# LucasAlegre/morl-baselines

Hardware: NVIDIA H100
Metric: envelope_q_updates_per_sec (higher is better)
Workload: dtype f32

## Files before the change

include/morl_b200.h:

```cpp
#ifndef MORL_B200_H_
#define MORL_B200_H_

#include <stddef.h>
#include <stdint.h>

#ifdef __cplusplus
extern "C" {
#endif

#define MORL_B200_VERSION 100

#if defined(__GNUC__)
#define MORL_API __attribute__((visibility("default")))
#else
#define MORL_API
#endif

#define MORL_OK 0
#define MORL_ERR_NULL (-1)
#define MORL_ERR_SHAPE (-2)
#define MORL_ERR_ALIGN (-3)
#define MORL_ERR_UNSUPPORTED (-4)
#define MORL_ERR_NO_DEVICE (-5)

// ... 110 lines not shown
MORL_API int morl_gemm_planes_f32(int fmt, const void* a_planes, long long a_plane_stride, const float* a_scale, const void* b_planes,
                                  long long b_plane_stride, const float* b_scale, int M, int N, int N_pad, int K, const float* bias,
                                  int relu, const void* relu_mask_plane0, int ld_mask, float* c_f32, int ldc, void* c_planes, int ldp,
                                  long long c_plane_stride, const float* c_scale, int reverse_tiles, int split_accumulators,
                                  const void* relu_bits_in, void* relu_bits_out, void* stream);
MORL_API int morl_gemm_planes_ln_f32(int fmt, const void* a_planes, long long a_plane_stride, const float* a_scale, const void* b_planes,
                                     long long b_plane_stride, const float* b_scale, int M, int N, int K, const float* bias, int layer_norm,
                                     const float* ln_gamma, const float* ln_beta, float ln_eps, float drop_p, const unsigned long long* drop_seed,
                                     const unsigned int* drop_offset, unsigned int drop_salt, float* c_f32, int ldc, void* c_planes, int ldp,
                                     long long c_plane_stride, const float* c_scale, int reverse_tiles, void* drop_bits_out, void* stream);
MORL_API int morl_philox_advance(unsigned int* offset, unsigned int inc, void* stream);
MORL_API int morl_gemm_chain_supported(int fmt, int M, int K);
MORL_API int morl_gemm_chain_f32(int fmt, int n_chains, int n_layers, const void* const* act_planes, long long act_plane_stride, const float* act_scale,
                                 const void* const* w_planes, long long w_plane_stride, const float* const* w_scales, const float* const* biases,
                                 int relu, const void* const* relu_bits_in, void* const* relu_bits_out, int M, int K, int k_first, void* stream);
MORL_API int morl_debug_gemm_stats(unsigned long long* out8, int reset);
MORL_API int morl_ensemble_sample_f32(const float* out, const float* max_logvar, const float* min_logvar, const int32_t* model_idx, const float* noise,
                                      const float* obs, int rew_dim, int E, int N, int O, float* sample_out, float* var_out, float* uncertainty_out,
                                      void* stream);

MORL_API int morl_qhead_envelope_supported(int fmt, int B, int W, int A, int D, int K);
MORL_API int morl_qhead_gemm_supported(int fmt, int M, int N, int K);
MORL_API int morl_qhead_gemm_f32(int fmt, const void* a_planes, long long a_plane_stride, const float* a_scale, const void* w_planes,
                                 long long w_plane_stride, const float* w_scale, const float* bias, int M, int N, int K, int reverse_tiles,
                                 float* q_out, void* stream);
MORL_API int morl_qhead_envelope_td_f32(int fmt, const void* a_on_planes, const void* a_tg_planes, long long a_plane_stride,
                                        const float* a_scale_on, const float* a_scale_tg, const void* w_on_planes, const void* w_tg_planes,
                                        long long w_plane_stride, const float* w_scale_on, const float* w_scale_tg, const float* bias_on,
                                        const float* bias_tg, int K, const float* wset, const float* reward, const float* done, float gamma,
                                        int B, int W, int A, int D, int dot_mode, int row_order, int reverse_tiles, float* target_out,
// ... 37 lines not shown
```

morl_baselines_b200/_lib.py:

```python

from __future__ import annotations

import ctypes as C
import os

HERE = os.path.dirname(os.path.abspath(__file__))
LIB_PATH = os.path.join(HERE, "csrc", "libmorl_b200.so")

DOT_UNFUSED, DOT_FMA, DOT_PAIRFMA = 0, 1, 2
MAP_TILE, MAP_BLOCK = 0, 1
ROWS_REFERENCE, ROWS_BMAJOR = 0, 1
AC_ELEMENTWISE_MIN, AC_SCALAR_MIN, AC_ARGMIN_GATHER = 0, 1, 2
MAX_D = 8
FMT_BF16X3, FMT_F16X2 = 0, 1

_vp, _i, _f, _d, _i64, _sz = C.c_void_p, C.c_int, C.c_float, C.c_double, C.c_int64, C.c_size_t

SIGNATURES = {
    "morl_version": (_i, []),
    "morl_last_error": (C.c_char_p, []),
    "morl_device_sm_count": (_i, []),
    "morl_envelope_td_f32": (_i, [_vp, _vp, _vp, _vp, _vp, _f, _i, _i, _i, _i, _i, _i, _vp, _vp, _vp, _vp]),
    "morl_greedy_td_f32": (_i, [_vp, _vp, _vp, _i, _i, _vp, _vp, _i, _i, _f, _i, _i, _i, _i, _vp, _vp, _vp]),
    "morl_critic_min_td_f32": (_i, [_vp, _i, _vp, _i, _i, _vp, _vp, _i, _i, _f, _i, _i, _i, _i, _vp, _vp, _vp]),
# ... 20 lines not shown
    "morl_front_unpack_f64": (_i, [_vp, _i, _i, _i, _i, _vp, _vp, _vp]),
    "morl_hypervolume_f64": (_i, [_vp, _vp, _i, _i, _vp, _vp, _vp]),
    "morl_corner_weights_f64": (_i, [_vp, _i, _i, _vp, _i, _vp, _vp]),
    "morl_polyak_f32": (_i, [_vp, _vp, _vp, _i, _i64, _d, _vp]),
    "morl_plane_overflow_count": (_i, [_i]),
    "morl_amax_scale_f32": (_i, [_vp, C.c_longlong, _i, _vp, _vp, _vp]),
    "morl_split_planes_multi": (_i, [_i, _vp, _i, _vp]),
    "morl_split_planes": (_i, [_i, _vp, _i, _i, _i, _i, _vp, _i, _i, C.c_longlong, _vp, _vp]),
    "morl_gemm_planes_f32": (_i, [_i, _vp, C.c_longlong, _vp, _vp, C.c_longlong, _vp, _i, _i, _i, _i, _vp, _i, _vp, _i, _vp, _i, _vp, _i, C.c_longlong,
                                  _vp, _i, _i, _vp, _vp, _vp]),
    "morl_gemm_planes_ln_f32": (_i, [_i, _vp, C.c_longlong, _vp, _vp, C.c_longlong, _vp, _i, _i, _i, _vp, _i, _vp, _vp, _f, _f, _vp, _vp, C.c_uint,
                                     _vp, _i, _vp, _i, C.c_longlong, _vp, _i, _vp, _vp]),
    "morl_philox_advance": (_i, [_vp, C.c_uint, _vp]),
    "morl_gemm_chain_supported": (_i, [_i, _i, _i]),
    "morl_gemm_chain_f32": (_i, [_i, _i, _i, _vp, C.c_longlong, _vp, _vp, C.c_longlong, _vp, _vp, _i, _vp, _vp, _i, _i, _i, _vp]),
    "morl_debug_gemm_stats": (_i, [_vp, _i]),
    "morl_ensemble_sample_f32": (_i, [_vp, _vp, _vp, _vp, _vp, _vp, _i, _i, _i, _i, _vp, _vp, _vp, _vp]),
    "morl_qhead_envelope_supported": (_i, [_i, _i, _i, _i, _i, _i]),
    "morl_qhead_gemm_supported": (_i, [_i, _i, _i, _i]),
    "morl_qhead_gemm_f32": (_i, [_i, _vp, C.c_longlong, _vp, _vp, C.c_longlong, _vp, _vp, _i, _i, _i, _i, _vp, _vp]),
    "morl_qhead_envelope_td_f32": (_i, [_i, _vp, _vp, C.c_longlong, _vp, _vp, _vp, _vp, C.c_longlong, _vp, _vp, _vp, _vp, _i, _vp, _vp, _vp, _f, _i, _i,
                                        _i, _i, _i, _i, _i, _vp, _vp, _vp, _vp, _vp, _vp]),
    "morl_pairs_relu_split_planes": (_i, [_i, _vp, _vp, _i, _i, _i, _vp, C.c_longlong, _vp, _vp, _vp]),
    "morl_pairs_product_split_planes": (_i, [_i, _vp, _vp, _i, _i, _i, _vp, C.c_longlong, _vp, _vp]),
    "morl_gemm_mn_workspace_bytes": (_sz, [_i, _i, _i]),
    "morl_gemm_planes_mn_f32": (_i, [_i, _vp, C.c_longlong, _i, _i, _vp, _vp, C.c_longlong, _i, _i, _vp, _i, _i, _vp, _i, _vp, _vp, _vp]),
    "morl_colsum_planes": (_i, [_i, _vp, C.c_longlong, _vp, _i, _i, _i, _vp, _vp, _vp]),
    "morl_pairs_grad_reduce_planes": (_i, [_i, _vp, C.c_longlong, _vp, _i, _i, _i, _vp, _vp, _vp, _vp]),
    "morl_pair_layer1_uv_f32": (_i, [_vp, _vp, _vp, _vp, _i, _i, _i, _i, _i, _vp, _vp, _vp]),
    "morl_product_layer1_uv_f32": (_i, [_vp, _vp, _vp, _i, _i, _vp, _vp, _vp, _i, _i, _i, _vp, _vp, _vp]),
# ... 45 lines not shown
```

morl_baselines_b200/csrc/gemm_planes.cu:

```cuda
#include <cuda.h>
#include <cuda_bf16.h>
#include <cuda_fp16.h>
#include <stdlib.h>
#include <string.h>

#include "common.cuh"
#include "gemm_tc.cuh"

namespace morl {

constexpr int kGemmBM = 128;
constexpr int kGemmThreads = 384;
constexpr int kGemmConsumerRegs = 232, kGemmProducerRegs = 40;
constexpr int kGemmBoxN = 32;

__device__ unsigned int g_plane_overflow;


__device__ __forceinline__ void note_overflow(float amax) {
    if (amax > 65504.f) atomicAdd(&g_plane_overflow, 1u);
}

#define MORL_DISPATCH_FMT(F_, ...)                                                         \
    switch (F_) {                                                                          \
// ... 163 lines not shown
    float k_acc;
    float c_mul;
    const float* bias_s;
    int relu;
    const uint32_t* bits_in;
    uint32_t* bits_out;
    int bits_ld;
    const uint16_t* mask;
    int ld_mask;
    float* c_f32;
    int ldc;
    int planes;
    int ldp;
};

template <int FMT, bool PRE = false>
__device__ __forceinline__ void epilogue_chunk(const float (&a)[16], int col0, int rbase, int lane, const EpiArgs& e, const CUtensorMap* tmC,
                                               uint8_t* my_stage, uint32_t& n_stored, float& amax) {
    using F = PlaneFmt<FMT>;
    constexpr int P = F::P;
    const int l4 = lane & 3, lr = lane >> 2;
    const int wi = relu_bits_word(col0);
    float x[2][8];
#pragma unroll
    for (int h = 0; h < 2; ++h)
#pragma unroll
        for (int q = 0; q < 4; ++q)
#pragma unroll
            for (int c = 0; c < 2; ++c) {
                float f;
                if constexpr (PRE) f = a[4 * q + 2 * h + c];
                else f = __fmaf_rn(a[4 * q + 2 * h + c], e.k_acc, e.bias_s[col0 + 8 * q + 2 * l4 + c]);
                if (e.relu) f = (f < 0.f) ? 0.f : f;
                x[h][2 * q + c] = f;
            }
    if (e.bits_in) {
#pragma unroll
        for (int h = 0; h < 2; ++h) {
            const int row = rbase + lr + 8 * h;
            const uint32_t keep = row < e.M ? __ldg(e.bits_in + (size_t)row * e.bits_ld + wi) : 0u;
#pragma unroll
            for (int j = 0; j < 8; ++j)
                if (!((keep >> (8 * (j >> 1) + 2 * l4 + (j & 1))) & 1u)) x[h][j] = 0.f;
        }
    }
    if (e.bits_out) {
#pragma unroll
        for (int h = 0; h < 2; ++h) {
            const int row = rbase + lr + 8 * h;
            uint32_t positive = 0;
#pragma unroll
            for (int j = 0; j < 8; ++j)
                if (x[h][j] > 0.f) positive |= 1u << (8 * (j >> 1) + 2 * l4 + (j & 1));
            positive |= __shfl_xor_sync(0xffffffffu, positive, 1);
            positive |= __shfl_xor_sync(0xffffffffu, positive, 2);
            if (l4 == 0 && row < e.M) e.bits_out[(size_t)row * e.bits_ld + wi] = positive;
        }
    }
    if (e.mask) {
#pragma unroll
        for (int h = 0; h < 2; ++h) {
            const int row = rbase + lr + 8 * h;
            if (row < e.M) {
#pragma unroll
                for (int q = 0; q < 4; ++q) {
                    const uint32_t mm = __ldg(reinterpret_cast<const uint32_t*>(e.mask + (size_t)row * e.ld_mask + col0 + 8 * q + 2 * l4));
                    if ((mm & 0x8000u) || (mm & 0x7FFFu) == 0u) x[h][2 * q] = 0.f;
                    if ((mm & 0x80000000u) || (mm & 0x7FFF0000u) == 0u) x[h][2 * q + 1] = 0.f;
                }
            }
        }
    }
    if (e.c_f32) {
// ... 354 lines not shown
                    e.k_acc = s_act / (s_act * ld_scale(g.b_scale[job]));
                    e.c_mul = 1.0f;
                    e.bias_s = s.bias; e.relu = g.relu; e.bits_in = g.bits_in[job]; e.bits_out = g.bits_out[job]; e.bits_ld = relu_bits_words(BN);
                    e.mask = nullptr; e.ld_mask = 0;
                    e.c_f32 = nullptr; e.ldc = 0; e.planes = 1; e.ldp = BN;
                    const int rbase = tile * kGemmBM + wg * 64 + (warp & 3) * 16;
                    consume_unit<FMT, 0, false>(acc, s, ring, l == 0 ? n_kblk_first : n_kblk_full, 0, BN, rbase, wg, lane, nullptr, [] {}, e,
                                                &maps.C[job], my_stage, n_stored, amax);
                    __syncwarp();
                    if (lane == 0) {
                        asm volatile("cp.async.bulk.wait_group 0;" ::: "memory");
                        g_mbar_arrive(&stored[ln]);
                    }
                }
        if (FMT == MORL_FMT_F16X2) note_overflow(amax);
    }
}

constexpr int kMnKT = 32;

__device__ __forceinline__ uint64_t make_desc_mn_sw128(uint32_t smem_addr, uint32_t lbo_bytes) {
    uint64_t d = 0;
    d |= (uint64_t)((smem_addr >> 4) & 0x3FFF);
    d |= (uint64_t)((lbo_bytes >> 4) & 0x3FFF) << 16;
    d |= (uint64_t)(1024 >> 4) << 32;
    d |= (uint64_t)1 << 62;
    return d;
}

struct GemmMnArgs {
// ... 1079 lines not shown
    a.thr = t >= 4294967295.0 ? 4294967295u : (unsigned int)t;
    a.scale = (float)(1.0 / (1.0 - (double)drop_p));
    a.bits = drop_bits_out;
    return gemm_planes_impl(fmt, a_planes, a_plane_stride, a_scale, b_planes, b_plane_stride, b_scale, M, N, N, K, bias, 1, nullptr, 0, c_f32, ldc,
                            c_planes, ldp, c_plane_stride, c_scale, reverse_tiles, 0, nullptr, nullptr, &a, "morl_gemm_planes_ln_f32", stream);
}

extern "C" int morl_philox_advance(unsigned int* offset, unsigned int inc, void* stream) {
    using namespace morl;
    MORL_REQUIRE(offset, MORL_ERR_NULL, "morl_philox_advance: NULL pointer argument");
    launch_k(philox_advance_kernel, dim3(1), dim3(1), 0, static_cast<cudaStream_t>(stream), offset, inc);
    return check_launch("morl_philox_advance");
}


extern "C" int morl_gemm_chain_supported(int fmt, int M, int K) {
    using namespace morl;
    return fmt_ok(fmt) && M >= 2 * kGemmBM && K == 256;
}

extern "C" int morl_gemm_chain_f32(int fmt, int n_chains, int n_layers, const void* const* act_planes, long long act_plane_stride, const float* act_scale,
                                   const void* const* w_planes, long long w_plane_stride, const float* const* w_scales, const float* const* biases,
                                   int relu, const void* const* relu_bits_in, void* const* relu_bits_out, int M, int K, int k_first, void* stream) {
    using namespace morl;
    MORL_REQUIRE(act_planes && w_planes, MORL_ERR_NULL, "morl_gemm_chain_f32: NULL pointer argument");
    MORL_REQUIRE(n_chains >= 1 && n_chains <= 2 && n_layers >= 1 && n_chains * n_layers <= kChainMaxJobs, MORL_ERR_SHAPE,
                 "morl_gemm_chain_f32: need 1 <= n_chains <= 2 and n_chains * n_layers <= %d (got %d x %d)", kChainMaxJobs, n_chains, n_layers);
    MORL_REQUIRE(morl_gemm_chain_supported(fmt, M, K), MORL_ERR_UNSUPPORTED, "morl_gemm_chain_f32: unsupported configuration fmt=%d M=%d K=%d (256-wide layers, M >= 256)",
                 fmt, M, K);
    const int BK = fmt_bk(fmt);
    if (k_first <= 0) k_first = K;
    MORL_REQUIRE(k_first % BK == 0 && k_first <= K, MORL_ERR_SHAPE, "morl_gemm_chain_f32: k_first=%d must be a multiple of %d and <= K", k_first, BK);
    ChainMaps maps;
    ChainArgs g;
    memset(&g, 0, sizeof(g));
    g.M = M; g.K = K; g.k_first = k_first; g.n_chains = n_chains; g.n_layers = n_layers; g.a_scale = act_scale; g.relu = relu ? 1 : 0;
    for (int c = 0; c < n_chains; ++c)
        for (int l = 0; l < n_layers; ++l) {
            const int job = c * n_layers + l;
            const void* a_in = act_planes[c * (n_layers + 1) + l];
            const void* a_out = act_planes[c * (n_layers + 1) + l + 1];
            MORL_REQUIRE(a_in && a_out && w_planes[job] && aligned16(a_in) && aligned16(a_out) && aligned16(w_planes[job]), MORL_ERR_NULL,
                         "morl_gemm_chain_f32: NULL or misaligned plane pointer (chain %d, layer %d)", c, l);
            const int kj = l == 0 ? k_first : K;
            const long long a_stride = l == 0 ? (long long)M * k_first : act_plane_stride;
            const long long w_stride = l == 0 ? (long long)256 * k_first : w_plane_stride;
            int rc = make_plane_map(&maps.A[job], fmt, a_in, M, kj, a_stride, kGemmBM, BK);
// ... 7 lines not shown
            g.bits_out[job] = relu_bits_out ? static_cast<uint32_t*>(relu_bits_out[job]) : nullptr;
            g.bits_in[job] = relu_bits_in ? static_cast<const uint32_t*>(relu_bits_in[job]) : nullptr;
            MORL_REQUIRE(aligned16(g.bits_out[job]) && aligned16(g.bits_in[job]), MORL_ERR_ALIGN, "morl_gemm_chain_f32: ReLU bit masks must be 16-byte aligned");
        }
    const int sms = sm_count();
    const int n_tiles = (M + kGemmBM - 1) / kGemmBM;
    MORL_DISPATCH_FMT(fmt, {
        constexpr size_t smem = KPlan<kFmt>::kBytes;
        g.n_stages = KPlan<kFmt>::kStages;
        set_smem_limit_once<gemm_chain_kernel<kFmt>>(smem);
        launch_k_pdl(gemm_pdl_enabled(), gemm_chain_kernel<kFmt>, dim3(n_tiles < sms ? n_tiles : sms), dim3(kGemmThreads), smem,
                     static_cast<cudaStream_t>(stream), maps, g);
    });
    return check_launch("morl_gemm_chain_f32");
}
```

morl_baselines_b200/multi_policy/envelope/envelope.py:

```python

from __future__ import annotations

import os
from typing import List, Optional, Union

import numpy as np
import torch as th
import torch.nn as nn
import torch.optim as optim

from ... import ops
from ...tc_mlp import TCPairMlp, TCPairMlpFn
from ...common.buffer import ReplayBuffer
from ...common.fused_adam import FusedClipAdam
from ...common.morl_algorithm import MOAgent, MOPolicy
from ...common.networks import NatureCNN, get_grad_norm, layer_init, mlp, polyak_update
from ...common.prioritized_buffer import PrioritizedReplayBuffer
from ...common.utils import linearly_decaying_value
from ...common.weights import equally_spaced_weights, random_weights

_FUSED_HEAD = os.environ.get("MORL_FUSED_HEAD", "1") != "0"
_PRE_REFRESH = os.environ.get("MORL_PRE_REFRESH", "1") == "1"
_HEAD_REVERSE = os.environ.get("MORL_HEAD_REVERSE", "1") == "1"
_DEFER_TREE = os.environ.get("MORL_DEFER_TREE", "1") != "0"
# ... 319 lines not shown
                else:
                    TCPairMlp.refresh_many([self._tc_on, self._tc_tg], transposed_of=[self._tc_train] if self._tc_train is not None else [])
                early_q = None
                if _THREE_STREAMS and self._tc_train is not None:
                    main, side3 = th.cuda.current_stream(), s["side_stream3"]
                    side3.wait_stream(main)
                    with th.cuda.stream(side3):
                        dp_ = self._dp
                        ws_ = wset if dp_ is None else wset[dp_["rank"] * dp_["w_loc"] : (dp_["rank"] + 1) * dp_["w_loc"]]
                        early_q = self._tc_train.forward_pairs(obs, ws_)
                fused_head = self.envelope and _FUSED_HEAD and self.tensor_core_accumulators != "split" and self._tc_on.head_operands() is not None \
                    and ops.qhead_envelope_supported(self._tc_fmt, B, W, A, D, self._tc_on.lin[-1].in_features)
                self.fused_head_active = bool(fused_head)
                head_reverse = False
                if fused_head:
                    if self._tc_on.chain_supported() and self._tc_tg.chain_supported():
                        if self._nograd_chain is None:
                            self._nograd_chain = TCPairMlp.make_chain([self._tc_on, self._tc_tg])
                        self._tc_on.layer1(nobs, wset)
                        self._tc_tg.layer1(nobs, wset)
                        self._nograd_chain()
                        h_on, h_tg = self._tc_on.h[-1], self._tc_tg.h[-1]
                        head_reverse = _HEAD_REVERSE
                    elif _TWO_STREAMS:
                        main, side = th.cuda.current_stream(), s["side_stream2"]
                        side.wait_stream(main)
                        with th.cuda.stream(side):
                            h_tg = self._tc_tg.forward_hidden(nobs, wset)
                        h_on = self._tc_on.forward_hidden(nobs, wset)
                        main.wait_stream(side)
                    else:
# ... 422 lines not shown
```

morl_baselines_b200/ops.py:

```python

from __future__ import annotations

from typing import Optional, Tuple

import torch as th

from . import _lib
from ._lib import (
    AC_ARGMIN_GATHER,
    AC_ELEMENTWISE_MIN,
    AC_SCALAR_MIN,
    DOT_FMA,
    DOT_PAIRFMA,
    DOT_UNFUSED,
    MAP_BLOCK,
    MAP_TILE,
    ROWS_BMAJOR,
    ROWS_REFERENCE,
)

launch_count = 0


def _count(n=1):
# ... 589 lines not shown
            if t is not None and (t.dtype != th.int32 or tuple(t.shape) != (self.M, relu_bits_words(self.N)) or not t.is_contiguous()):
                raise _lib.MorlB200Error(f"GemmChain: ReLU bit masks must be contiguous int32 [{self.M}, {relu_bits_words(self.N)}]")
        self._keep = (flat_a, flat_w, flat_b, flat_s, flat_m, flat_i, act_scale)
        self.relu = bool(relu)
        arr = lambda ts: (C.c_void_p * len(ts))(*[None if t is None else t.data_ptr() for t in ts])
        self._pa, self._pw, self._pb, self._ps, self._pm, self._pi = arr(flat_a), arr(flat_w), arr(flat_b), arr(flat_s), arr(flat_m), arr(flat_i)
        self._a_stride, self._w_stride, self._act_scale = a0.stride(0), 256 * self.K, act_scale

    def __call__(self):
        rc = _lib.load().morl_gemm_chain_f32(self.fmt, self.n_chains, self.n_layers, self._pa, self._a_stride, _ptr(self._act_scale), self._pw, self._w_stride,
                                             self._ps, self._pb, int(self.relu), self._pi, self._pm, self.M, self.K, self.k_first, _stream())
        _lib.check(rc, "morl_gemm_chain_f32")
        _count()


def qhead_gemm_supported(fmt: int, M: int, N: int, K: int) -> bool:
    return bool(_lib.load().morl_qhead_gemm_supported(int(fmt), int(M), int(N), int(K)))


def qhead_gemm(a_planes: th.Tensor, w_planes: th.Tensor, n_out: int, bias: th.Tensor, out: Optional[th.Tensor] = None, a_scale=None, w_scale=None,
               reverse_tiles: bool = False) -> th.Tensor:
    fmt = fmt_of(a_planes)
    _, M, K = a_planes.shape
    if fmt_of(w_planes) != fmt or tuple(w_planes.shape[1:]) != (32, K) or a_planes.stride(1) != K or w_planes.stride(1) != K:
        raise _lib.MorlB200Error(f"qhead_gemm: need K-major planes A [P, M, K] and W [P, 32, K] of one format (got {tuple(a_planes.shape)}, {tuple(w_planes.shape)})")
    if out is None:
        out = th.empty((M, n_out), device=a_planes.device, dtype=th.float32)
    rc = _lib.load().morl_qhead_gemm_f32(fmt, _ptr(a_planes), a_planes.stride(0), _ptr(a_scale), _ptr(w_planes), w_planes.stride(0), _ptr(w_scale), _ptr(bias), M,
                                         n_out, K, int(reverse_tiles), _ptr(out), _stream())
    _lib.check(rc, "morl_qhead_gemm_f32")
# ... 169 lines not shown
```

morl_baselines_b200/tc_mlp.py:

```python

from __future__ import annotations

import os
from typing import List, Optional

import torch as th
from torch import nn

from . import ops

_SNAKE = os.environ.get("MORL_TC_SNAKE", "1") == "1"
_CHAIN = os.environ.get("MORL_GEMM_CHAIN", "1") == "1"
_CHAIN_BWD = os.environ.get("MORL_GEMM_CHAIN_BWD", "1") == "1"
_NARROW_HEAD = os.environ.get("MORL_NARROW_HEAD", "1") == "1"
_DEFAULT_FMT = ops.FMT_BF16X3 if os.environ.get("MORL_TC_FMT", "f16x2") == "bf16x3" else ops.FMT_F16X2

MAX_HIDDEN = 512
MAX_TRAIN_W = 256
ACT_SCALE = 2.0
W_TARGET_EXP = 14
G_TARGET_EXP = 2


def _pad(n: int, m: int) -> int:
# ... 137 lines not shown
                                   reverse_tiles=_SNAKE and bool(k & 1), a_scale=self.s_act, b_scale=self.s_w[k - 1], c_scale=self.s_act,
                                   split_acc=self.split_acc, relu_bits_out=hb[k])
        return a

    def chain_supported(self) -> bool:
        hid = [l.out_features for l in self.lin[:-1]]
        return (_CHAIN and not self.split_acc and len(hid) >= 2 and all(h == 256 for h in hid)
                and ops.gemm_chain_supported(self.fmt, self.B * self.W, 256))

    def layer1(self, feats: th.Tensor, wset: th.Tensor) -> th.Tensor:
        first = self.lin[0]
        u, v = ops.pair_layer1_uv(feats, wset, first.weight.detach(), first.bias.detach())
        hb = self.hbits if self.trainable else [None] * len(self.h)
        return ops.pairs_relu_split(u, v, out=self.h[0], scale=self.s_act, relu_bits_out=hb[0])

    def chain_spec(self):
        n = len(self.lin)
        hb = self.hbits if self.trainable else [None] * len(self.h)
        return (list(self.h), [self.wp[k - 1] for k in range(1, n - 1)], [self.lin[k].bias for k in range(1, n - 1)],
                [self.s_w[k - 1] for k in range(1, n - 1)], [hb[k] for k in range(1, n - 1)])

    @staticmethod
    def make_chain(plans):
        specs = [p.chain_spec() for p in plans]
        return ops.GemmChain([sp[0] for sp in specs], [sp[1] for sp in specs], [sp[2] for sp in specs], [sp[3] for sp in specs],
                             [sp[4] for sp in specs], act_scale=plans[0].s_act)

    def head_operands(self):
        last = self.lin[-1]
        wp = self.wp[len(self.lin) - 2]
# ... 208 lines not shown
```

Before: 693.7.

## Fuse pair-expansion layer into a shared-memory-resident GEMM chain kernel

Adds a persistent chain kernel that builds the first hidden activation (relu(u[b]+v[j])) directly in shared memory from the per-observation and per-weight partial products, then runs all hidden 256-wide layers with the activation kept resident in shared memory. Only the last layer's output is written to global memory. This removes the separate pairs_relu_split pass and the global write and reload of intermediate activation planes. It is used on the no-grad target path when the format is f16x2. In exchange it adds a large new kernel with a 3-stage weight ring and extra shared-memory pressure.

```diff
diff --git a/include/morl_b200.h b/include/morl_b200.h
--- a/include/morl_b200.h
+++ b/include/morl_b200.h
@@ -148,6 +148,10 @@
 MORL_API int morl_gemm_chain_f32(int fmt, int n_chains, int n_layers, const void* const* act_planes, long long act_plane_stride, const float* act_scale,
                                  const void* const* w_planes, long long w_plane_stride, const float* const* w_scales, const float* const* biases,
                                  int relu, const void* const* relu_bits_in, void* const* relu_bits_out, int M, int K, int k_first, void* stream);
+MORL_API int morl_gemm_chain_pairs_f32(int n_chains, int n_layers, const float* const* u, const float* const* v, int B, int W, const void* const* acts,
+                                       long long act_plane_stride, const float* act_scale, const void* const* w_planes, long long w_plane_stride,
+                                       const float* const* w_scales, const float* const* biases, void* const* relu_bits_out, unsigned int store_mask,
+                                       void* stream);
 MORL_API int morl_debug_gemm_stats(unsigned long long* out8, int reset);
 MORL_API int morl_ensemble_sample_f32(const float* out, const float* max_logvar, const float* min_logvar, const int32_t* model_idx, const float* noise,
                                       const float* obs, int rew_dim, int E, int N, int O, float* sample_out, float* var_out, float* uncertainty_out,
diff --git a/morl_baselines_b200/_lib.py b/morl_baselines_b200/_lib.py
--- a/morl_baselines_b200/_lib.py
+++ b/morl_baselines_b200/_lib.py
@@ -58,6 +58,7 @@
     "morl_philox_advance": (_i, [_vp, C.c_uint, _vp]),
     "morl_gemm_chain_supported": (_i, [_i, _i, _i]),
     "morl_gemm_chain_f32": (_i, [_i, _i, _i, _vp, C.c_longlong, _vp, _vp, C.c_longlong, _vp, _vp, _i, _vp, _vp, _i, _i, _i, _vp]),
+    "morl_gemm_chain_pairs_f32": (_i, [_i, _i, _vp, _vp, _i, _i, _vp, C.c_longlong, _vp, _vp, C.c_longlong, _vp, _vp, _vp, C.c_uint, _vp]),
     "morl_debug_gemm_stats": (_i, [_vp, _i]),
     "morl_ensemble_sample_f32": (_i, [_vp, _vp, _vp, _vp, _vp, _vp, _i, _i, _i, _i, _vp, _vp, _vp, _vp]),
     "morl_qhead_envelope_supported": (_i, [_i, _i, _i, _i, _i, _i]),
diff --git a/morl_baselines_b200/csrc/gemm_planes.cu b/morl_baselines_b200/csrc/gemm_planes.cu
--- a/morl_baselines_b200/csrc/gemm_planes.cu
+++ b/morl_baselines_b200/csrc/gemm_planes.cu
@@ -201,49 +201,55 @@
     int ldp;
 };
 
+template <bool PRE>
+__device__ __forceinline__ void epilogue_values(const float (&a)[16], int col0, int rbase, int lane, const EpiArgs& e, float (&x)[2][8]) {
+    const int l4 = lane & 3, lr = lane >> 2;
+    const int wi = relu_bits_word(col0);
+#pragma unroll
+    for (int h = 0; h < 2; ++h)
+#pragma unroll
+        for (int q = 0; q < 4; ++q)
+#pragma unroll
+            for (int c = 0; c < 2; ++c) {
+                float f;
+                if constexpr (PRE) f = a[4 * q + 2 * h + c];
+                else f = __fmaf_rn(a[4 * q + 2 * h + c], e.k_acc, e.bias_s[col0 + 8 * q + 2 * l4 + c]);
+                if (e.relu) f = (f < 0.f) ? 0.f : f;
+                x[h][2 * q + c] = f;
+            }
+    if (e.bits_in) {
+#pragma unroll
+        for (int h = 0; h < 2; ++h) {
+            const int row = rbase + lr + 8 * h;
+            const uint32_t keep = row < e.M ? __ldg(e.bits_in + (size_t)row * e.bits_ld + wi) : 0u;
+#pragma unroll
+            for (int j = 0; j < 8; ++j)
+                if (!((keep >> (8 * (j >> 1) + 2 * l4 + (j & 1))) & 1u)) x[h][j] = 0.f;
+        }
+    }
+    if (e.bits_out) {
+#pragma unroll
+        for (int h = 0; h < 2; ++h) {
+            const int row = rbase + lr + 8 * h;
+            uint32_t positive = 0;
+#pragma unroll
+            for (int j = 0; j < 8; ++j)
+                if (x[h][j] > 0.f) positive |= 1u << (8 * (j >> 1) + 2 * l4 + (j & 1));
+            positive |= __shfl_xor_sync(0xffffffffu, positive, 1);
+            positive |= __shfl_xor_sync(0xffffffffu, positive, 2);
+            if (l4 == 0 && row < e.M) e.bits_out[(size_t)row * e.bits_ld + wi] = positive;
+        }
+    }
+}
+
 template <int FMT, bool PRE = false>
 __device__ __forceinline__ void epilogue_chunk(const float (&a)[16], int col0, int rbase, int lane, const EpiArgs& e, const CUtensorMap* tmC,
                                                uint8_t* my_stage, uint32_t& n_stored, float& amax) {
     using F = PlaneFmt<FMT>;
     constexpr int P = F::P;
     const int l4 = lane & 3, lr = lane >> 2;
-    const int wi = relu_bits_word(col0);
     float x[2][8];
-#pragma unroll
-    for (int h = 0; h < 2; ++h)
-#pragma unroll
-        for (int q = 0; q < 4; ++q)
-#pragma unroll
-            for (int c = 0; c < 2; ++c) {
-                float f;
-                if constexpr (PRE) f = a[4 * q + 2 * h + c];
-                else f = __fmaf_rn(a[4 * q + 2 * h + c], e.k_acc, e.bias_s[col0 + 8 * q + 2 * l4 + c]);
-                if (e.relu) f = (f < 0.f) ? 0.f : f;
-                x[h][2 * q + c] = f;
-            }
-    if (e.bits_in) {
-#pragma unroll
-        for (int h = 0; h < 2; ++h) {
-            const int row = rbase + lr + 8 * h;
-            const uint32_t keep = row < e.M ? __ldg(e.bits_in + (size_t)row * e.bits_ld + wi) : 0u;
-#pragma unroll
-            for (int j = 0; j < 8; ++j)
-                if (!((keep >> (8 * (j >> 1) + 2 * l4 + (j & 1))) & 1u)) x[h][j] = 0.f;
-        }
-    }
-    if (e.bits_out) {
-#pragma unroll
-        for (int h = 0; h < 2; ++h) {
-            const int row = rbase + lr + 8 * h;
-            uint32_t positive = 0;
-#pragma unroll
-            for (int j = 0; j < 8; ++j)
-                if (x[h][j] > 0.f) positive |= 1u << (8 * (j >> 1) + 2 * l4 + (j & 1));
-            positive |= __shfl_xor_sync(0xffffffffu, positive, 1);
-            positive |= __shfl_xor_sync(0xffffffffu, positive, 2);
-            if (l4 == 0 && row < e.M) e.bits_out[(size_t)row * e.bits_ld + wi] = positive;
-        }
-    }
+    epilogue_values<PRE>(a, col0, rbase, lane, e, x);
     if (e.mask) {
 #pragma unroll
         for (int h = 0; h < 2; ++h) {
@@ -628,6 +634,298 @@
                     }
                 }
         if (FMT == MORL_FMT_F16X2) note_overflow(amax);
+    }
+}
+
+struct ResPlan {
+    static constexpr int P = 2, BK = 32, kStages = 3;
+    static constexpr uint32_t kRowB = BK * 2;
+    static constexpr uint32_t kKBlock = P * kGemmBM * kRowB;
+    static constexpr uint32_t kPlaneKB = kGemmBM * kRowB;
+    static constexpr uint32_t kAct = 8 * kKBlock;
+    static constexpr uint32_t kBStage = P * 256 * kRowB;
+    static constexpr uint32_t kOffB = kAct;
+    static constexpr uint32_t kOffBias = kOffB + kStages * kBStage;
+    static constexpr uint32_t kOffBar = kOffBias + 1024;
+    static constexpr uint32_t kBytes = kOffBar + 256 + 1024;
+    static_assert(kBytes <= 232448, "dynamic shared memory of one CTA on sm_90 (227 KB)");
+};
+
+struct alignas(64) ResChainMaps {
+    CUtensorMap A[2];
+    CUtensorMap B[kChainMaxJobs];
+    CUtensorMap C[kChainMaxJobs];
+};
+
+struct ResChainArgs {
+    int M, K, k_first, n_chains, n_layers;
+    const float* bias[kChainMaxJobs];
+    const float* b_scale[kChainMaxJobs];
+    uint32_t* bits_out[kChainMaxJobs];
+    const uint32_t* bits_in[kChainMaxJobs];
+    const float* a_scale;
+    int relu;
+    uint32_t store;
+    const float* u[2];
+    const float* v[2];
+    int W;
+    unsigned long long* stats;
+};
+
+__device__ __forceinline__ void mma_unit_resident(float (&acc)[128], uint32_t act, const KSmem& s, Ring& ring, int n_kblk, int wg, int lane,
+                                                  long long* wait_cycles) {
+    using F = PlaneFmt<MORL_FMT_F16X2>;
+    using R = ResPlan;
+    constexpr uint32_t b_plane = 256u * R::kRowB;
+    const uint32_t a_wg = act + (uint32_t)wg * 64u * R::kRowB;
+    uint32_t prev = 0;
+    for (int kb = 0; kb < n_kblk; ++kb) {
+        const long long c0 = wait_cycles ? clock64() : 0;
+        g_mbar_wait(&s.full[ring.stage], ring.phase);
+        if (wait_cycles) *wait_cycles += clock64() - c0;
+        wgmma_fence();
+        const uint32_t a0 = a_wg + (uint32_t)kb * R::kKBlock;
+        const uint32_t b0 = g_smem_u32(s.b + ring.stage * R::kBStage);
+#pragma unroll
+        for (int ks = 0; ks < R::BK / 16; ++ks) {
+#pragma unroll
+            for (int t = 0; t < F::NPROD; ++t) {
+                const uint64_t ad = make_desc_k<R::kRowB>(a0 + F::pa(t) * R::kPlaneKB + ks * 32);
+                const uint64_t bd = make_desc_k<R::kRowB>(b0 + F::pb(t) * b_plane + ks * 32);
+                Wgmma<256>::template mma<MORL_FMT_F16X2, 0, 0>(acc, ad, bd, (kb | ks | t) != 0 ? 1u : 0u);
+            }
+        }
+        wgmma_commit();
+        if (kb > 0) {
+            wgmma_wait<1>();
+            if (lane == 0) g_mbar_arrive(&s.empty[prev]);
+        }
+        prev = ring.stage;
+        ring.advance();
+    }
+    wgmma_wait<0>();
+    if (n_kblk > 0 && lane == 0) g_mbar_arrive(&s.empty[prev]);
+}
+
+__device__ __forceinline__ uint8_t* res_chunk(uint8_t* act, int kb, int row, int q) {
+    return act + (uint32_t)kb * ResPlan::kKBlock + (uint32_t)row * ResPlan::kRowB + (uint32_t)((q ^ ((row >> 1) & 3)) << 4);
+}
+
+__global__ void __launch_bounds__(kGemmThreads, 1)
+gemm_chain_resident_kernel(const __grid_constant__ ResChainMaps maps, const ResChainArgs g) {
+    using F = PlaneFmt<MORL_FMT_F16X2>;
+    using R = ResPlan;
+    constexpr int P = R::P, BN = 256;
+    extern __shared__ uint8_t gsmem_raw[];
+    uint8_t* sm = align_1k(gsmem_raw);
+    uint8_t* act = sm;
+    KSmem s;
+    s.a = nullptr;
+    s.b = sm + R::kOffB;
+    s.b_stage = R::kBStage;
+    s.c = nullptr;
+    s.bias = reinterpret_cast<float*>(sm + R::kOffBias);
+    s.full = reinterpret_cast<uint64_t*>(sm + R::kOffBar);
+    s.empty = s.full + R::kStages;
+    uint64_t* act_full = s.empty + R::kStages;
+    uint64_t* act_empty = act_full + 1;
+    const bool pairs = g.u[0] != nullptr;
+
+    const int warp = threadIdx.x >> 5;
+    const int lane = threadIdx.x & 31;
+    const int unit = blockIdx.x, n_units = gridDim.x;
+    const int n_tiles = (g.M + kGemmBM - 1) / kGemmBM;
+    const int n_kblk_full = g.K / R::BK, n_kblk_first = g.k_first / R::BK;
+    const int cu0 = unit, cu1 = (unit + n_units / 2) % n_units;
+    const int mt0 = cu0 < n_tiles ? (n_tiles - cu0 + n_units - 1) / n_units : 0;
+    const int mt1 = g.n_chains > 1 ? (cu1 < n_tiles ? (n_tiles - cu1 + n_units - 1) / n_units : 0) : 0;
+    const int n_ti = mt0 > mt1 ? mt0 : mt1;
+    auto tile_row = [&](int ti, int c) { return ti < (c ? mt1 : mt0) ? ((c ? cu1 : cu0) + ti * n_units) * kGemmBM : -1; };
+
+    if (threadIdx.x == 0) {
+        init_ring_barriers(s.full, s.empty, R::kStages);
+        g_mbar_init(act_full, 1);
+        g_mbar_init(act_empty, 8);
+        g_mbar_init_fence();
+    }
+    pdl_enter();
+    __syncthreads();
+
+    if (warp >= 8) {
+        warpgroup_reg_dec<kGemmProducerRegs>();
+        if (warp == 8 && lane == 0) {
+            Ring ring((uint32_t)R::kStages);
+            long long w_empty = 0;
+            uint32_t n_in = 0;
+            for (int ti = 0; ti < n_ti; ++ti)
+                for (int c = 0; c < g.n_chains; ++c) {
+                    const int row0 = tile_row(ti, c);
+                    if (row0 < 0) continue;
+                    for (int l = 0; l < g.n_layers; ++l) {
+                        const int job = c * g.n_layers + l;
+                        const int nkb = l == 0 ? n_kblk_first : n_kblk_full;
+                        for (int kb = 0; kb < nkb; ++kb) {
+                            if (!pairs && l == 0 && kb == (nkb < R::kStages ? nkb - 1 : R::kStages - 1)) {
+                                if (n_in > 0) {
+                                    const long long c0 = g.stats ? clock64() : 0;
+                                    g_mbar_wait(act_empty, (n_in - 1u) & 1u);
+                                    if (g.stats) w_empty += clock64() - c0;
+                                }
+                                g_mbar_expect_tx(act_full, (uint32_t)n_kblk_first * R::kKBlock);
+                                for (int k = 0; k < n_kblk_first; ++k) tma_load_3d(act + k * R::kKBlock, &maps.A[c], act_full, k * R::BK, row0, 0);
+                                ++n_in;
+                            }
+                            const long long c0 = g.stats ? clock64() : 0;
+                            g_mbar_wait(&s.empty[ring.stage], ring.phase ^ 1u);
+                            if (g.stats) w_empty += clock64() - c0;
+                            uint64_t* full = &s.full[ring.stage];
+                            g_mbar_expect_tx(full, R::kBStage);
+                            uint8_t* bs = s.b + ring.stage * R::kBStage;
+                            for (int p = 0; p < P; ++p) tma_load_3d(bs + (uint32_t)p * 256u * R::kRowB, &maps.B[job], full, kb * R::BK, 0, p);
+                            ring.advance();
+                        }
+                    }
+                }
+            if (g.stats) atomicAdd(&g.stats[2], (unsigned long long)w_empty);
+        }
+    } else {
+        warpgroup_reg_inc<kGemmConsumerRegs>();
+        const int wg = warp >> 2, wr = warp & 3;
+        const int l4 = lane & 3, lr = lane >> 2;
+        const int trow = wg * 64 + wr * 16;
+        const float s_act = ld_scale(g.a_scale);
+        const uint32_t act_s = g_smem_u32(act);
+        float amax = 0.f;
+        float acc[128];
+        Ring ring((uint32_t)R::kStages);
+        long long w_full = 0, busy = 0, w_act = 0;
+        const long long t_begin = g.stats ? clock64() : 0;
+        uint32_t n_in = 0;
+        for (int ti = 0; ti < n_ti; ++ti)
+            for (int c = 0; c < g.n_chains; ++c) {
+                const int row0 = tile_row(ti, c);
+                if (row0 < 0) continue;
+                if (pairs) {
+                    if (lane == 0) asm volatile("cp.async.bulk.wait_group.read 0;" ::: "memory");
+                    __syncwarp();
+                    const float* u = c ? g.u[1] : g.u[0];
+                    const float* v = c ? g.v[1] : g.v[0];
+#pragma unroll
+                    for (int h = 0; h < 2; ++h) {
+                        const int rl = trow + lr + 8 * h, row = row0 + rl;
+                        const bool ok = row < g.M;
+                        const int b = ok ? row / g.W : 0, j = ok ? row - b * g.W : 0;
+#pragma unroll 2
+                        for (int kb = 0; kb < 8; ++kb) {
+                            const int col = kb * 32 + 8 * l4;
+                            uint32_t o[P][4];
+                            if (ok) {
+                                const float4* up = reinterpret_cast<const float4*>(u + (size_t)b * BN + col);
+                                const float4* vp = reinterpret_cast<const float4*>(v + (size_t)j * BN + col);
+                                const float4 u0 = __ldg(up), u1 = __ldg(up + 1), v0 = __ldg(vp), v1 = __ldg(vp + 1);
+                                const float x[8] = {u0.x + v0.x, u0.y + v0.y, u0.z + v0.z, u0.w + v0.w, u1.x + v1.x, u1.y + v1.y, u1.z + v1.z, u1.w + v1.w};
+#pragma unroll
+                                for (int t = 0; t < 4; ++t) {
+                                    uint32_t w[P];
+                                    const float r0 = x[2 * t] < 0.f ? 0.f : x[2 * t], r1 = x[2 * t + 1] < 0.f ? 0.f : x[2 * t + 1];
+                                    F::split2(r0 * s_act, r1 * s_act, w, amax);
+#pragma unroll
+                                    for (int p = 0; p < P; ++p) o[p][t] = w[p];
+                                }
+                            } else {
+#pragma unroll
+                                for (int t = 0; t < 4; ++t)
+#pragma unroll
+                                    for (int p = 0; p < P; ++p) o[p][t] = 0u;
+                            }
+                            uint8_t* dst = res_chunk(act, kb, rl, l4);
+#pragma unroll
+                            for (int p = 0; p < P; ++p) *reinterpret_cast<uint4*>(dst + p * R::kPlaneKB) = make_uint4(o[p][0], o[p][1], o[p][2], o[p][3]);
+                        }
+                    }
+                    asm volatile("fence.proxy.async.shared::cta;" ::: "memory");
+                    bar_sync_named(2 + wg, 128);
+                }
+                for (int l = 0; l < g.n_layers; ++l) {
+                    const int job = c * g.n_layers + l;
+                    const bool last = l == g.n_layers - 1, store = (g.store >> job) & 1u;
+                    reload_bias(s.bias, g.bias[job], 0, BN, s_act);
+                    if (!pairs && l == 0) {
+                        const long long c0 = g.stats ? clock64() : 0;
+                        g_mbar_wait(act_full, n_in & 1u);
+                        if (g.stats) w_act += clock64() - c0;
+                    }
+                    mma_unit_resident(acc, act_s, s, ring, l == 0 ? n_kblk_first : n_kblk_full, wg, lane, g.stats ? &w_full : nullptr);
+                    const long long c1 = g.stats ? clock64() : 0;
+                    EpiArgs e;
+                    e.M = g.M; e.N = BN;
+                    e.k_acc = s_act / (s_act * ld_scale(g.b_scale[job]));
+                    e.c_mul = 1.0f;
+                    e.bias_s = s.bias; e.relu = g.relu; e.bits_in = g.bits_in[job]; e.bits_out = g.bits_out[job]; e.bits_ld = relu_bits_words(BN);
+                    e.mask = nullptr; e.ld_mask = 0; e.c_f32 = nullptr; e.ldc = 0; e.planes = 1; e.ldp = BN;
+                    const bool to_tile = !last || store;
+                    if (to_tile) {
+                        if (lane == 0) asm volatile("cp.async.bulk.wait_group.read 0;" ::: "memory");
+                        __syncwarp();
+                    }
+                    const int rbase = row0 + trow;
+#pragma unroll
+                    for (int cc = 0; cc < 8; ++cc) {
+                        float a[16];
+#pragma unroll
+                        for (int jj = 0; jj < 16; ++jj) a[jj] = acc[16 * cc + jj];
+                        float x[2][8];
+                        epilogue_values<false>(a, 32 * cc, rbase, lane, e, x);
+                        if (to_tile) {
+#pragma unroll
+                            for (int h = 0; h < 2; ++h) {
+                                const int rl = lr + 8 * h;
+#pragma unroll
+                                for (int q = 0; q < 4; ++q) {
+                                    uint32_t w[P];
+                                    F::split2(x[h][2 * q], x[h][2 * q + 1], w, amax);
+                                    uint8_t* st = res_chunk(act, cc, trow + rl, q) + 4 * l4;
+#pragma unroll
+                                    for (int p = 0; p < P; ++p) *reinterpret_cast<uint32_t*>(st + p * R::kPlaneKB) = w[p];
+                                }
+                            }
+                            if (store) {
+                                asm volatile("fence.proxy.async.shared::cta;" ::: "memory");
+                                __syncwarp();
+                                if (lane == 0) {
+                                    const uint32_t src = act_s + (uint32_t)cc * R::kKBlock + (uint32_t)trow * R::kRowB;
+#pragma unroll
+                                    for (int p = 0; p < P; ++p)
+                                        asm volatile("cp.async.bulk.tensor.3d.global.shared::cta.bulk_group [%0, {%2, %3, %4}], [%1];" ::"l"(&maps.C[job]),
+                                                     "r"(src + p * R::kPlaneKB), "r"(32 * cc), "r"(rbase), "r"(p)
+                                                     : "memory");
+                                    asm volatile("cp.async.bulk.commit_group;" ::: "memory");
+                                }
+                            }
+                        }
+                    }
+                    if (!last) {
+                        asm volatile("fence.proxy.async.shared::cta;" ::: "memory");
+                        bar_sync_named(2 + wg, 128);
+                    } else if (!pairs) {
+                        __syncwarp();
+                        if (lane == 0) {
+                            asm volatile("cp.async.bulk.wait_group.read 0;" ::: "memory");
+                            g_mbar_arrive(act_empty);
+                        }
+                    }
+                    if (g.stats) busy += clock64() - c1;
+                }
+                ++n_in;
+            }
+        if (g.stats && warp == 0 && lane == 0) {
+            atomicAdd(&g.stats[0], (unsigned long long)w_full);
+            atomicAdd(&g.stats[1], (unsigned long long)(clock64() - t_begin));
+            atomicAdd(&g.stats[3], (unsigned long long)busy);
+            atomicAdd(&g.stats[4], (unsigned long long)w_act);
+        }
+        note_overflow(amax);
+        if (lane == 0) asm volatile("cp.async.bulk.wait_group 0;" ::: "memory");
     }
 }
 
@@ -1737,6 +2035,57 @@
 }
 
 
+namespace morl {
+static int launch_chain_resident(ResChainArgs& g, int n_chains, int n_layers, const void* const* in, const void* const* acts, long long act_plane_stride,
+                                 const float* act_scale, const void* const* w_planes, long long w_plane_stride, const float* const* w_scales,
+                                 const float* const* biases, int relu, const void* const* relu_bits_in, void* const* relu_bits_out, int M, int K,
+                                 const char* name, void* stream) {
+    constexpr int fmt = MORL_FMT_F16X2;
+    ResChainMaps maps;
+    memset(&maps, 0, sizeof(maps));
+    g.M = M; g.K = K; g.n_chains = n_chains; g.n_layers = n_layers; g.a_scale = act_scale; g.relu = relu ? 1 : 0;
+    for (int c = 0; c < n_chains; ++c) {
+        if (!g.u[0]) {
+            MORL_REQUIRE(in[c] && aligned16(in[c]), MORL_ERR_NULL, "%s: NULL or misaligned input planes (chain %d)", name, c);
+            const int rc = make_plane_map(&maps.A[c], fmt, in[c], M, g.k_first, (long long)M * g.k_first, kGemmBM, ResPlan::BK);
+            MORL_REQUIRE(rc == 0, MORL_ERR_NO_DEVICE, "%s: cuTensorMapEncodeTiled(A) failed (%d)", name, rc);
+        }
+        for (int l = 0; l < n_layers; ++l) {
+            const int job = c * n_layers + l;
+            const int kj = l == 0 ? g.k_first : K;
+            const long long w_stride = l == 0 ? (long long)256 * g.k_first : w_plane_stride;
+            MORL_REQUIRE(w_planes[job] && aligned16(w_planes[job]), MORL_ERR_NULL, "%s: NULL or misaligned weight planes (chain %d, layer %d)", name, c, l);
+            int rc = make_plane_map(&maps.B[job], fmt, w_planes[job], 256, kj, w_stride, 256, ResPlan::BK, true);
+            MORL_REQUIRE(rc == 0, MORL_ERR_NO_DEVICE, "%s: cuTensorMapEncodeTiled(B) failed (%d)", name, rc);
+            if ((g.store >> job) & 1u) {
+                const void* out = acts[c * (n_layers + 1) + l + 1];
+                MORL_REQUIRE(out && aligned16(out), MORL_ERR_NULL, "%s: NULL or misaligned output planes (chain %d, layer %d)", name, c, l);
+                rc = make_plane_map(&maps.C[job], fmt, out, M, 256, act_plane_stride, 16, 32, true);
+                MORL_REQUIRE(rc == 0, MORL_ERR_NO_DEVICE, "%s: cuTensorMapEncodeTiled(C) failed (%d)", name, rc);
+            }
+            g.bias[job] = biases ? biases[job] : nullptr;
+            g.b_scale[job] = w_scales ? w_scales[job] : nullptr;
+            g.bits_out[job] = relu_bits_out ? static_cast<uint32_t*>(relu_bits_out[job]) : nullptr;
+            g.bits_in[job] = relu_bits_in ? static_cast<const uint32_t*>(relu_bits_in[job]) : nullptr;
+            MORL_REQUIRE(aligned16(g.bits_out[job]) && aligned16(g.bits_in[job]), MORL_ERR_ALIGN, "%s: ReLU bit masks must be 16-byte aligned", name);
+        }
+    }
+    static const bool want_stats = [] { const char* e = getenv("MORL_GEMM_STATS"); return e && e[0] == '1'; }();
+    if (want_stats) {
+        void* sp = nullptr;
+        cudaGetSymbolAddress(&sp, g_gemm_stats);
+        g.stats = static_cast<unsigned long long*>(sp);
+    }
+    const int sms = sm_count();
+    const int n_tiles = (M + kGemmBM - 1) / kGemmBM;
+    constexpr size_t smem = ResPlan::kBytes;
+    set_smem_limit_once<gemm_chain_resident_kernel>(smem);
+    launch_k_pdl(gemm_pdl_enabled(), gemm_chain_resident_kernel, dim3(n_tiles < sms ? n_tiles : sms), dim3(kGemmThreads), smem,
+                 static_cast<cudaStream_t>(stream), maps, g);
+    return check_launch(name);
+}
+}
+
 extern "C" int morl_gemm_chain_supported(int fmt, int M, int K) {
     using namespace morl;
     return fmt_ok(fmt) && M >= 2 * kGemmBM && K == 256;
@@ -1751,9 +2100,19 @@
                  "morl_gemm_chain_f32: need 1 <= n_chains <= 2 and n_chains * n_layers <= %d (got %d x %d)", kChainMaxJobs, n_chains, n_layers);
     MORL_REQUIRE(morl_gemm_chain_supported(fmt, M, K), MORL_ERR_UNSUPPORTED, "morl_gemm_chain_f32: unsupported configuration fmt=%d M=%d K=%d (256-wide layers, M >= 256)",
                  fmt, M, K);
-    const int BK = fmt_bk(fmt);
+    const int BK = fmt == MORL_FMT_F16X2 ? ResPlan::BK : fmt_bk(fmt);
     if (k_first <= 0) k_first = K;
     MORL_REQUIRE(k_first % BK == 0 && k_first <= K, MORL_ERR_SHAPE, "morl_gemm_chain_f32: k_first=%d must be a multiple of %d and <= K", k_first, BK);
+    if (fmt == MORL_FMT_F16X2) {
+        ResChainArgs g;
+        memset(&g, 0, sizeof(g));
+        g.k_first = k_first;
+        g.store = (1u << (n_chains * n_layers)) - 1u;
+        const void* in[2] = {nullptr, nullptr};
+        for (int c = 0; c < n_chains; ++c) in[c] = act_planes[c * (n_layers + 1)];
+        return launch_chain_resident(g, n_chains, n_layers, in, act_planes, act_plane_stride, act_scale, w_planes, w_plane_stride, w_scales, biases,
+                                     relu, relu_bits_in, relu_bits_out, M, K, "morl_gemm_chain_f32", stream);
+    }
     ChainMaps maps;
     ChainArgs g;
     memset(&g, 0, sizeof(g));
@@ -1791,3 +2150,32 @@
     });
     return check_launch("morl_gemm_chain_f32");
 }
+
+extern "C" int morl_gemm_chain_pairs_f32(int n_chains, int n_layers, const float* const* u, const float* const* v, int B, int W, const void* const* acts,
+                                         long long act_plane_stride, const float* act_scale, const void* const* w_planes, long long w_plane_stride,
+                                         const float* const* w_scales, const float* const* biases, void* const* relu_bits_out, unsigned int store_mask,
+                                         void* stream) {
+    using namespace morl;
+    MORL_REQUIRE(u && v && w_planes, MORL_ERR_NULL, "morl_gemm_chain_pairs_f32: NULL pointer argument");
+    MORL_REQUIRE(n_chains >= 1 && n_chains <= 2 && n_layers >= 1 && n_chains * n_layers <= kChainMaxJobs, MORL_ERR_SHAPE,
+                 "morl_gemm_chain_pairs_f32: need 1 <= n_chains <= 2 and n_chains * n_layers <= %d (got %d x %d)", kChainMaxJobs, n_chains, n_layers);
+    MORL_REQUIRE(B > 0 && W > 0 && (long long)B * W <= 0x7fffffffLL && morl_gemm_chain_supported(MORL_FMT_F16X2, B * W, 256), MORL_ERR_SHAPE,
+                 "morl_gemm_chain_pairs_f32: bad shape B=%d W=%d (need B W >= 256)", B, W);
+    MORL_REQUIRE(store_mask < (1u << (n_chains * n_layers)), MORL_ERR_SHAPE, "morl_gemm_chain_pairs_f32: store_mask 0x%x names jobs beyond %d x %d", store_mask,
+                 n_chains, n_layers);
+    MORL_REQUIRE(store_mask == 0 || acts, MORL_ERR_NULL, "morl_gemm_chain_pairs_f32: stored outputs need their planes");
+    ResChainArgs g;
+    memset(&g, 0, sizeof(g));
+    g.k_first = 256;
+    g.store = store_mask;
+    g.W = W;
+    const void* outs[2 * (kChainMaxJobs + 1)] = {};
+    for (int c = 0; c < n_chains; ++c) {
+        MORL_REQUIRE(u[c] && v[c] && aligned16(u[c]) && aligned16(v[c]), MORL_ERR_ALIGN, "morl_gemm_chain_pairs_f32: u / v of chain %d NULL or not 16-byte aligned", c);
+        g.u[c] = u[c];
+        g.v[c] = v[c];
+        for (int l = 0; l < n_layers; ++l) outs[c * (n_layers + 1) + l + 1] = acts ? acts[c * n_layers + l] : nullptr;
+    }
+    return launch_chain_resident(g, n_chains, n_layers, nullptr, outs, act_plane_stride, act_scale, w_planes, w_plane_stride, w_scales, biases, 1, nullptr,
+                                 relu_bits_out, B * W, 256, "morl_gemm_chain_pairs_f32", stream);
+}
diff --git a/morl_baselines_b200/multi_policy/envelope/envelope.py b/morl_baselines_b200/multi_policy/envelope/envelope.py
--- a/morl_baselines_b200/multi_policy/envelope/envelope.py
+++ b/morl_baselines_b200/multi_policy/envelope/envelope.py
@@ -357,7 +357,15 @@
                 self.fused_head_active = bool(fused_head)
                 head_reverse = False
                 if fused_head:
-                    if self._tc_on.chain_supported() and self._tc_tg.chain_supported():
+                    if self._tc_on.pair_chain_supported() and self._tc_tg.pair_chain_supported():
+                        if self._nograd_chain is None:
+                            self._nograd_chain = TCPairMlp.make_pair_chain([self._tc_on, self._tc_tg])
+                        u_on, v_on = self._tc_on.layer1_uv(nobs, wset)
+                        u_tg, v_tg = self._tc_tg.layer1_uv(nobs, wset)
+                        self._nograd_chain([u_on, u_tg], [v_on, v_tg])
+                        h_on, h_tg = self._tc_on.h[-1], self._tc_tg.h[-1]
+                        head_reverse = _HEAD_REVERSE
+                    elif self._tc_on.chain_supported() and self._tc_tg.chain_supported():
                         if self._nograd_chain is None:
                             self._nograd_chain = TCPairMlp.make_chain([self._tc_on, self._tc_tg])
                         self._tc_on.layer1(nobs, wset)
diff --git a/morl_baselines_b200/ops.py b/morl_baselines_b200/ops.py
--- a/morl_baselines_b200/ops.py
+++ b/morl_baselines_b200/ops.py
@@ -627,6 +627,56 @@
         _count()
 
 
+class GemmChainPairs:
+
+    def __init__(self, outs, weights, B: int, W: int, biases=None, w_scales=None, bits=None, act_scale=None):
+        import ctypes as C
+
+        self.n_chains, self.n_layers = len(outs), len(weights[0])
+        self.B, self.W, self.M = int(B), int(W), int(B) * int(W)
+        flat_o = [t for ch in outs for t in ch]
+        flat_w = [t for ch in weights for t in ch]
+        flat_b = [None] * len(flat_w) if biases is None else [t.detach() for ch in biases for t in ch]
+        flat_s = [None] * len(flat_w) if w_scales is None else [t for ch in w_scales for t in ch]
+        flat_m = [None] * len(flat_w) if bits is None else [t for ch in bits for t in ch]
+        if len(flat_o) != len(flat_w) or any(len(w) != self.n_layers for w in weights) or any(len(o) != self.n_layers for o in outs):
+            raise _lib.MorlB200Error("GemmChainPairs: every chain needs n_layers outputs (or None) and n_layers weight tensors")
+        for t in flat_w:
+            if fmt_of(t) != FMT_F16X2 or tuple(t.shape[1:]) != (256, 256) or not t.is_contiguous():
+                raise _lib.MorlB200Error("GemmChainPairs: weight planes must be contiguous f16x2 [2, 256, 256]")
+        stored = [t for t in flat_o if t is not None]
+        for t in stored:
+            if fmt_of(t) != FMT_F16X2 or tuple(t.shape[1:]) != (self.M, 256) or not t.is_contiguous() or not t.is_cuda:
+                raise _lib.MorlB200Error(f"GemmChainPairs: output planes must be contiguous CUDA f16x2 tensors [2, {self.M}, 256]")
+        if any(t.stride(0) != stored[0].stride(0) for t in stored):
+            raise _lib.MorlB200Error("GemmChainPairs: output planes need one plane stride")
+        for t in flat_m:
+            if t is not None and (t.dtype != th.int32 or tuple(t.shape) != (self.M, relu_bits_words(256)) or not t.is_contiguous()):
+                raise _lib.MorlB200Error(f"GemmChainPairs: ReLU bit masks must be contiguous int32 [{self.M}, {relu_bits_words(256)}]")
+        self.store = sum(1 << i for i, t in enumerate(flat_o) if t is not None)
+        self._keep = (flat_o, flat_w, flat_b, flat_s, flat_m, act_scale)
+        arr = lambda ts: (C.c_void_p * len(ts))(*[None if t is None else t.data_ptr() for t in ts])
+        self._po, self._pw, self._pb, self._ps, self._pm = arr(flat_o), arr(flat_w), arr(flat_b), arr(flat_s), arr(flat_m)
+        self._o_stride = stored[0].stride(0) if stored else 0
+        self._w_stride, self._act_scale = flat_w[0].stride(0), act_scale
+
+    def __call__(self, us, vs):
+        import ctypes as C
+
+        if len(us) != self.n_chains or len(vs) != self.n_chains:
+            raise _lib.MorlB200Error(f"GemmChainPairs: need u and v of {self.n_chains} chains")
+        for u, v in zip(us, vs):
+            if (u.dtype != th.float32 or v.dtype != th.float32 or tuple(u.shape) != (self.B, 256) or tuple(v.shape) != (self.W, 256)
+                    or not u.is_contiguous() or not v.is_contiguous() or not u.is_cuda or not v.is_cuda):
+                raise _lib.MorlB200Error(f"GemmChainPairs: u / v must be contiguous CUDA float32 [{self.B}, 256] / [{self.W}, 256]")
+        pu = (C.c_void_p * self.n_chains)(*[u.data_ptr() for u in us])
+        pv = (C.c_void_p * self.n_chains)(*[v.data_ptr() for v in vs])
+        rc = _lib.load().morl_gemm_chain_pairs_f32(self.n_chains, self.n_layers, pu, pv, self.B, self.W, self._po, self._o_stride, _ptr(self._act_scale),
+                                                   self._pw, self._w_stride, self._ps, self._pb, self._pm, self.store, _stream())
+        _lib.check(rc, "morl_gemm_chain_pairs_f32")
+        _count()
+
+
 def qhead_gemm_supported(fmt: int, M: int, N: int, K: int) -> bool:
     return bool(_lib.load().morl_qhead_gemm_supported(int(fmt), int(M), int(N), int(K)))
 
diff --git a/morl_baselines_b200/tc_mlp.py b/morl_baselines_b200/tc_mlp.py
--- a/morl_baselines_b200/tc_mlp.py
+++ b/morl_baselines_b200/tc_mlp.py
@@ -175,6 +175,20 @@
         hb = self.hbits if self.trainable else [None] * len(self.h)
         return ops.pairs_relu_split(u, v, out=self.h[0], scale=self.s_act, relu_bits_out=hb[0])
 
+    def layer1_uv(self, feats: th.Tensor, wset: th.Tensor):
+        first = self.lin[0]
+        return ops.pair_layer1_uv(feats, wset, first.weight.detach(), first.bias.detach())
+
+    def pair_chain_supported(self) -> bool:
+        return self.fmt == ops.FMT_F16X2 and self.chain_supported()
+
+    @staticmethod
+    def make_pair_chain(plans):
+        specs = [p.chain_spec() for p in plans]
+        outs = [[None] * (len(sp[0]) - 2) + [sp[0][-1]] for sp in specs]
+        return ops.GemmChainPairs(outs, [sp[1] for sp in specs], plans[0].B, plans[0].W, [sp[2] for sp in specs], [sp[3] for sp in specs],
+                                  act_scale=plans[0].s_act)
+
     def chain_spec(self):
         n = len(self.lin)
         hb = self.hbits if self.trainable else [None] * len(self.h)
```

Result: faster. 822.9 (median of 6 runs) (+18.6%).
